# lzhLab/kmcEx

Hardware: AMD Instinct MI355X
Metric: k-mers/s encoded (insert) + k-mers/s queried, k=31 nh=7; % HBM-BW roofline (higher is better)
Workload: dtype u64; 1 GPU; synthetic 100000000 distinct canonical 31-mers per GPU, D1 counts, insert then query (110000000 queries: all inserted k-mers shuffled, half reverse-complemented, +10% absent); k=31, nh=7, nb=5, ci=1, cs=1023, kmers_per_gpu=100000000

## Files before the change

### kmcex_amd/csrc/kernels.hip

```cpp
#include "launchers.h"
#include <cstdlib>

__constant__ u32 c_seeds[128] = {
	46757, 46769, 46771, 46807, 46811, 46817, 46819, 46829, 46831, 46853, 46861, 46867, 46877, 46889, 46901, 46919,
	46933, 46957, 46993, 46997, 47017, 47041, 47051, 47057, 47059, 47087, 47093, 47111, 47119, 47123, 47129, 47137,
	47143, 47147, 47149, 47161, 47189, 47207, 47221, 47237, 47251, 47269, 47279, 47287, 47293, 47297, 47303, 47309,
	47317, 47339, 47351, 47353, 47363, 47381, 47387, 47389, 47407, 47417, 47419, 47431, 47441, 47459, 47491, 47497,
	47501, 47507, 47513, 47521, 47527, 47533, 47543, 47563, 47569, 47581, 47591, 47599, 47609, 47623, 47629, 47639,
	47653, 47657, 47659, 47681, 47699, 47701, 47711, 47713, 47717, 47737, 47741, 47743, 47777, 47779, 47791, 47797,
	47807, 47809, 47819, 47837, 47843, 47857, 47869, 47881, 47903, 47911, 47917, 47933, 47939, 47947, 47951, 47963,
	47969, 47977, 47981, 48017, 48023, 48029, 48049, 48073, 48079, 48091, 48109, 48119, 48121, 48131, 48157, 48163};

template <int W> __device__ __forceinline__ void load_kmer(const u64 *base, u64 i, u64 *v)
{
#pragma unroll
	for (int w = 0; w < W; w++) v[w] = base[i * W + w];
}
template <int W> __device__ __forceinline__ void store_kmer(u64 *base, u64 i, const u64 *v)
{
#pragma unroll
	for (int w = 0; w < W; w++) base[i * W + w] = v[w];
}

template <int W> __device__ __forceinline__ void bloom_insert_pm(const Premixed<W> &pm, const StrGeom g, u32 *bits, const ModU64 md, int nhash)
// ... 1700 lines not shown

template <int PW> __device__ __forceinline__ int decode_array(const ModelDev &md, const StrGeom gf, const Premixed<PW> &pf, int a)
{
	if (!md.km_mod.d) return -1;
	const cell_t *cells = md.cells[a];
	int v = 0;
	bool ok = true;
	for (int j = 0; j < md.nh && ok; j++) {
		u64 pos = mod_u64(murmur_seeded<PW>(pf, gf, c_seeds[(a * md.nh + j) & 127]), md.km_mod);
		const cell_t cell = cells[pos >> 4];
		u32 b = bit_in_cell(pos);
		ok = (cell >> (16 + b)) & 1u;
		v |= (int)((cell >> b) & 1u) << j;
	}
	return ok ? v : -1;
}

template <int PW> __device__ __forceinline__ int candidate_from_filters(const ModelDev &md, const StrGeom gf, const StrGeom gb, const Premixed<PW> &pf, const Premixed<PW> &pb)
{
	int occ = check_all_bf<PW>(md, gf, gb, pf, pb);
	if (occ != 0) return occ;
	if (bloom_check_pm<PW>(pb, gb, md.km_back, md.km_back_mod, md.nh - 2)) {
		int result = -1;
		for (int a = 0; a < md.nb; a++) {
			int d = decode_array<PW>(md, gf, pf, a);
			if (d >= 0) { result = d; if (d != 0) break; }
		}
		if (result > -1) return result;
	}
	return -2;
}

template <int PW, typename NEIGH>
__device__ __forceinline__ int occ_from_filters(const ModelDev &md, const StrGeom gf, const StrGeom gb, const Premixed<PW> &pf, const Premixed<PW> &pb, NEIGH neighbours)
{
	const bool in_back = bloom_check_pm<PW>(pb, gb, md.km_back, md.km_back_mod, md.nh - 2);
	const int occ = check_all_bf<PW>(md, gf, gb, pf, pb);
	if (!in_back) return occ;
	int nv = 0, first = 0;
	for (int a = 0; a < md.nb; a++) {
		int d = decode_array<PW>(md, gf, pf, a);
		if (d > 0) { if (nv == 0) first = d; nv++; }
	}
	int bin;
	if (nv == 0) bin = occ;
	else if (nv == 1) {
		bin = first;
		if (occ) {
			int cand[8];
			int nc = neighbours(cand), cnt = 0;
			for (int c = 0; c < 8; c++) cnt += (c < nc && cand[c] < md.ci + md.bf_num) ? 1 : 0;
			if (cnt >= nc / 2) bin = occ;
		}
	} else {
		int cand[8];
		int nc = neighbours(cand);
		if (nc <= 0) bin = 0;
		else {
			int min_dist = 2 << 20;
			bin = first;
			for (int a = 0; a < md.nb; a++) {
				int d = decode_array<PW>(md, gf, pf, a);
				if (d <= 0) continue;
				int cur = 2 << 20;
				for (int c = 0; c < 8; c++)
					if (c < nc) { int dd = d > cand[c] ? d - cand[c] : cand[c] - d; cur = dd < cur ? dd : cur; }
				if (min_dist > cur) { min_dist = cur; bin = d; }
			}
		}
	}
	return bin < (1 << md.nh) ? (int)md.mean_of_bin[bin] : 0;
}

template <int W> __device__ __forceinline__ int neighbour_candidate(const ModelDev &md, u64 *nv)
{
	min_kmer<W>(nv, md.k);
	int r = rest_check<W>(md, nv);
	if (r > 0) return (int)md.bin_of_occ[r];
	Aligned<W> al = left_align<W>(nv, md.k);
	Premixed<W> pf = premix_string<W>(al, md.gfull);
	Premixed<W> pb = premix_string<W>(drop_first_base<W>(al), md.gback);
	return candidate_from_filters<W>(md, md.gfull, md.gback, pf, pb);
}

template <int W> __device__ __forceinline__ int neighbour_bins(const ModelDev &md, const u64 *v, int *cand)
{
	int nc = 0;
	const int k = md.k;
	for (int x = 0; x < 8; x++) {
		u64 nv[W];
		if (x < 4) {
			if (W == 1) nv[0] = ((v[0] << 2) | (u64)x) & (k == 32 ? ~0ULL : ((1ULL << (2 * k)) - 1));
			else {
				nv[0] = ((v[0] << 2) | (v[W - 1] >> 62)) & (k == 64 ? ~0ULL : ((1ULL << (2 * k - 64)) - 1));
				nv[W - 1] = (v[W - 1] << 2) | (u64)x;
			}
		} else {
			u64 X = (u64)(x - 4);
			if (W == 1) nv[0] = (v[0] >> 2) | (X << (2 * (k - 1)));
			else {
				nv[W - 1] = (v[W - 1] >> 2) | (v[0] << 62);
				nv[0] = (v[0] >> 2) | (X << (2 * (k - 1) - 64));
			}
		}
		int c = neighbour_candidate<W>(md, nv);
		if (c != -2) cand[nc++] = c;
	}
	return nc;
}

template <int W, bool ACCT> __device__ __forceinline__ void query_packed_one(const ModelDev &md, u64 *v, u64 *acct, int *dst)
{
	if (md.k & 31) v[0] &= (1ULL << (2 * (md.k & 31))) - 1;
	min_kmer<W>(v, md.k);
	int occ = rest_check<W>(md, v);
	if (occ != 0) { *dst = occ; return; }
	Aligned<W> al = left_align<W>(v, md.k);
	Premixed<W> pf = premix_string<W>(al, md.gfull);
	Premixed<W> pb = premix_string<W>(drop_first_base<W>(al), md.gback);
	*dst = occ_from_filters<W>(md, md.gfull, md.gback, pf, pb, [&](int *cand) { if (ACCT) atomicAdd(acct, 1ULL); return neighbour_bins<W>(md, v, cand); });
}

template <int W, bool ACCT> __global__ __launch_bounds__(256) void k_query(ModelDev md, const u64 *kmers, u64 n, int *out, u64 *acct)
{
	const u64 q = (u64)blockIdx.x * 256 + threadIdx.x;
	if (q >= n) return;
	u64 v[W];
	load_kmer<W>(kmers, q, v);
	query_packed_one<W, ACCT>(md, v, acct, out + q);
}

struct AStr { u64 b[8]; };

__device__ __forceinline__ u32 code_of_byte(u32 c) { return c == 'C' ? 1u : (c == 'G' ? 2u : (c == 'T' ? 3u : 0u)); }

__device__ __forceinline__ void astr_codes(const AStr &s, int L, u64 &hi, u64 &lo)
{
	hi = lo = 0;
#pragma unroll
	for (int w = 0; w < 8; w++)
#pragma unroll
		for (int j = 0; j < 8; j++)
			if (8 * w + j < L) {
				const u32 c = code_of_byte((u32)(s.b[w] >> (8 * j)) & 0xFFu);
				hi = (hi << 2) | (lo >> 62);
				lo = (lo << 2) | c;
			}
}
__device__ __forceinline__ void astr_clip(AStr &s, int L)
{
#pragma unroll
	for (int w = 0; w < 8; w++) {
		const int keep = L - 8 * w;
// ... 669 lines not shown
		else hipLaunchKernelGGL((k_kmback_emit<2, 16, 2>), grid, blk, 0, st, md, bd, kmers, surv, i0, istride, pp, n_in_block, bs);
	}
}
void bs_apply(const BitScatter &bs, hipStream_t st)
{
	if (!bs.cap2) { hipLaunchKernelGGL(k_bs_apply, dim3(BS_BINS), dim3(1024), 0, st, bs); return; }
	const unsigned per_bin = (bs.cap + 256 * BS_SPLIT_K - 1) / (256 * BS_SPLIT_K);
	hipLaunchKernelGGL(k_bs_split, dim3(per_bin < 64 ? per_bin : 64, BS_BINS), dim3(256), 0, st, bs);
	hipLaunchKernelGGL(k_bs_apply2, dim3(1u << (bs.wshift - bs.tlog2), BS_BINS), dim3(1024), 0, st, bs);
}

void kmc_decode(const KmcDecode &d, int W_, u64 rec0, u64 n, u64 *kmers, u32 *counts, hipStream_t st)
{
	if (!n) return;
	DISPATCH_W(W_, hipLaunchKernelGGL(k_kmc_decode<W>, dim3((unsigned)((n + 255) / 256)), dim3(256), 0, st, d, rec0, n, kmers, counts));
}

void ring_import(const ModelDev &md, const BlockDev &bd, int pp, const RingLists &rl, u64 *stg_kmers, u32 *stg_counts, hipStream_t st)
{
	DISPATCH_W(words(md), hipLaunchKernelGGL(k_ring_import<W>, dim3(KMX_BUCKET / 256, md.nb), dim3(256), 0, st, bd, md.nb, pp, rl, stg_kmers, stg_counts));
}
void ring_export(const ModelDev &md, const BlockDev &bd, int pp, const RingLists &rl, u64 *feedback, hipStream_t st)
{
	DISPATCH_W(words(md), hipLaunchKernelGGL(k_ring_export<W>, dim3(KMX_BUCKET / 256, md.nb), dim3(256), 0, st, bd, pp, rl, feedback));
}
void or_words(u32 *dst, const u32 *src, u64 n, hipStream_t st)
{
	if (!n) return;
	u64 blocks = (n + 1023) / 1024;
	if (blocks > 65536) blocks = 65536;
	hipLaunchKernelGGL(k_or_words, dim3((unsigned)blocks), dim3(256), 0, st, dst, src, n);
}

void query(const ModelDev &md, const u64 *kmers, u64 n, int *out, hipStream_t st, KernelProf *prof, u64 *acct)
{
	if (!n) return;
	KPROF_BEGIN(prof, KC_QUERY, st);
	if (acct) DISPATCH_W(words(md), hipLaunchKernelGGL((k_query<W, true>), dim3((unsigned)((n + 255) / 256)), dim3(256), 0, st, md, kmers, n, out, acct));
	else DISPATCH_W(words(md), hipLaunchKernelGGL((k_query<W, false>), dim3((unsigned)((n + 255) / 256)), dim3(256), 0, st, md, kmers, n, out, (u64 *)nullptr));
	KPROF_END(prof, st);
}

void query_ascii(const ModelDev &md, int L, const unsigned char *strs, int stride, u64 n, int *out, hipStream_t st)
{
	if (!n) return;
	const StrGeom gf = make_geom(L), gb = make_geom(L >= 2 ? L - 2 : 0);
	DISPATCH_W(words(md), hipLaunchKernelGGL(k_query_ascii<W>, dim3((unsigned)((n + 255) / 256)), dim3(256), 0, st, md, gf, gb, L, strs, stride, n, out));
}

void query_seq(const ModelDev &md, const unsigned char *seq, u64 n_bases, const u64 *offs, u64 n_seqs, u64 p0, u64 n_win, int *out, u32 *dlist, u32 cap, u32 *dcnt, u32 *dcnt_next, hipStream_t st, KernelProf *prof)
{
	if (!n_win) return;
	KPROF_BEGIN(prof, KC_QUERY, st);
	const StrGeom gf = make_geom(md.k), gb = make_geom(md.k - 2);
	DISPATCH_W(words(md), hipLaunchKernelGGL(k_query_seq<W>, dim3((unsigned)((n_win + SEQ_BT - 1) / SEQ_BT)), dim3(SEQ_BT), 0, st, md, seq, n_bases, offs, n_seqs, p0, n_win, out, dlist, cap, dcnt));
	DISPATCH_W(words(md), hipLaunchKernelGGL(k_query_ascii_at<W>, dim3(SEQ_DIRTY_WGS), dim3(256), 0, st, md, gf, gb, seq, n_bases, p0, (const u32 *)dlist, cap, (const u32 *)dcnt, dcnt_next, out));
	KPROF_END(prof, st);
}

void seq_summary_init(SeqSummary *rec, u64 n_seqs, hipStream_t st, KernelProf *prof)
{
	if (!n_seqs) return;
	KPROF_BEGIN(prof, KC_QUERY, st);
	hipLaunchKernelGGL(k_seq_summary_init, dim3((unsigned)((n_seqs + 255) / 256)), dim3(256), 0, st, rec, n_seqs);
	KPROF_END(prof, st);
}
// ... 65 lines not shown
```

### kmcex_amd/csrc/kmx_api.hip

```cpp
#include "../../include/kmx.h"
#include "hip_owned.h"
#include "kmc_reader.h"
#include "launchers.h"
#include "reads_reader.h"
#include "strpack.h"

#include <algorithm>
#include <atomic>
#include <exception>
#include <new>
#include <cstdarg>
#include <cstdio>
#include <cstdlib>
#include <cstring>
#include <chrono>
#include <condition_variable>
#include <functional>
#include <memory>
#include <mutex>
#include <string>
#include <thread>
#include <type_traits>
#include <vector>
#include <dlfcn.h>
// ... 58 lines not shown
	for (int i = 0; i < e1 && i < mc; i++) bin_of_occ[i] = i;
	mean_of_bin.assign(e3, 0);
	for (int b = 0; b < e1; b++) mean_of_bin[b] = b;
	std::vector<char> seen(e3, 0);
	for (int i = e1; i < mc; i++) {
		u32 b = bin_of_occ[i];
		if (b < (u32)e3 && !seen[b]) { seen[b] = 1; if ((int)b >= e1) mean_of_bin[b] = mean_of_occ[i]; }
	}
	return 0;
}

static int kmx_occubin_impl(int cs, int nh, uint32_t *bin_of_occ, uint32_t *mean_of_bin)
{
	if (nh < 3 || nh > KMX_MAX_NH || cs < 1) return fail(KMX_E_ARG, "bad cs/nh");
	std::vector<u32> b, m;
	if (occubin_tables(cs, nh, b, m)) return fail(KMX_E_ARG, "cs=%d too small for nh=%d", cs, nh);
	memcpy(bin_of_occ, b.data(), b.size() * 4);
	memcpy(mean_of_bin, m.data(), m.size() * 4);
	return KMX_OK;
}

struct RestTable {
	int k = 0, pre_len = 0, map_size = 0, pre_buffer_size = 0, suff_group = 0;
	u64 suff_bin_size = 0, entries = 0;
	std::vector<int> hash2index, pre_buffer, count_bin;
	std::vector<unsigned char> suffix_bin;
	bool host_valid = false;
	DevBuf<int> d_h2i, d_pre, d_cnt;
	DevBuf<u64> d_suf;
	DevBuf<u64> d_sorted;
	int fbits = 0;
	DevBuf<u32> d_fine;
	DevBuf<u64> d_q;
	void reset_dev() { d_h2i.reset(); d_pre.reset(); d_cnt.reset(); d_suf.reset(); d_sorted.reset(); d_fine.reset(); d_q.reset(); }
};
static int rest_prefix_len(int k) { for (int i = 7; i >= 3; i--) if ((k - i) % 4 == 0) return i; return 3; }
static int check_model_k(int k)
{
	if (k < 4 || k > 64) return fail(KMX_E_ARG, "k=%d out of range [4,64]%s", k, k == 3 ? ": the reference's rest table is undefined at k = 3 (prefix of 7 bases, rest.hpp:78-83)" : "");
	return KMX_OK;
}

struct RestEnt { u64 w[2]; int c; };

enum { ST_EMPTY = 0, ST_BUILDING = 1, ST_READY = 2 };

struct kmx_model {
	int ci = 1, cs = 1023, nh = 7, nb = 5, k = 0, bf_num = 1, W = 1;
	int device = 0, state = ST_EMPTY;
	hipStream_t stream = nullptr;
	std::vector<u32> h_bin_of_occ, h_mean_of_bin;
	DevBuf<u32> d_bin_of_occ, d_mean_of_bin;
	u64 n_total = 0, n_km = 0, n_bf[3] = {0, 0, 0};
	u64 byte_bf[3] = {0, 0, 0}, byte_bf_back[3] = {0, 0, 0}, km_byte_size = 0, byte_km_back = 0, ncells = 0;
	DevBuf<u32> d_bloom;
	u64 bloom_words = 0, bf_woff[3] = {0, 0, 0}, bf_back_woff[3] = {0, 0, 0};
	u32 *d_bf[3] = {nullptr, nullptr, nullptr}, *d_bf_back[3] = {nullptr, nullptr, nullptr};
	DevBuf<u32> d_km_back;
	DevBuf<cell_t> d_cells[KMX_MAX_NB];
	RestTable rest;
	ModelDev md;
	DevBuf<u64> d_stg_kmers;
	DevBuf<u32> d_stg_counts;
	u64 stg_n = 0;
	BlockDev bd;
	DevBuf<unsigned char> d_block_scratch;
	int scratch_nb = 0, scratch_W = 0;
// ... 274 lines not shown
	m->n_km = m->n_total - nbf;
	m->km_byte_size = (m->n_km >> 4) * (u64)m->nh;
	m->byte_km_back = (m->n_km >> 4) * (u64)(m->nh - 2);
	m->ncells = (m->km_byte_size + 1) / 2;
}

static void fill_model_dev(kmx_model *m)
{
	ModelDev &md = m->md;
	memset(&md, 0, sizeof md);
	md.k = m->k; md.nh = m->nh; md.nb = m->nb; md.ci = m->ci; md.cs = m->cs; md.bf_num = m->bf_num;
	{
		const char *e = hook_env("KMX_NH_FIRST"), *e2 = hook_env("KMX_NH_SECOND");
		const int f = e ? atoi(e) : (2 * m->nh + 3) / 7, f2 = e2 ? atoi(e2) : (4 * m->nh + 3) / 7;
		md.nh_first = f < 1 ? 1 : (f > m->nh ? m->nh : f);
		md.nh_second = f2 < md.nh_first ? md.nh_first : (f2 > m->nh ? m->nh : f2);
	}
	md.gfull = make_geom(m->k);
	md.gback = make_geom(m->k - 2);
	for (int i = 0; i < 3; i++) {
		md.bf[i] = m->d_bf[i]; md.bf_mod[i] = make_mod(i < m->bf_num ? m->byte_bf[i] * 8 : 0);
		md.bf_back[i] = m->d_bf_back[i]; md.bf_back_mod[i] = make_mod(i < m->bf_num ? m->byte_bf_back[i] * 8 : 0);
	}
	md.km_back = m->d_km_back; md.km_back_mod = make_mod(m->byte_km_back * 8);
	md.kmb_direct = m->kmb_deferred ? 0 : 1;
	md.bloom_direct = m->blm_deferred ? 0 : 1;
	for (int i = 0; i < 3; i++) { md.bf_woff[i] = m->bf_woff[i]; md.bf_back_woff[i] = m->bf_back_woff[i]; }
	for (int a = 0; a < m->nb; a++) md.cells[a] = m->d_cells[a];
	md.km_mod = make_mod(m->km_byte_size * 8);
	md.bin_of_occ = m->d_bin_of_occ; md.mean_of_bin = m->d_mean_of_bin;
	md.rest_pre_len = m->rest.pre_len; md.rest_W = m->W; md.rest_entries = m->rest.entries;
	md.rest_h2i = m->rest.d_h2i; md.rest_pre = m->rest.d_pre; md.rest_suf = m->rest.d_suf; md.rest_cnt = m->rest.d_cnt;
	md.rest_fbits = m->rest.fbits; md.rest_fine = m->rest.d_fine; md.rest_q = m->rest.d_q;
}

static int alloc_arrays(kmx_model *m)
{
	m->rest.reset_dev();
	{
		u64 off = 0;
		for (int i = 0; i < 3; i++) {
			m->bf_woff[i] = off; off += i < m->bf_num ? (m->byte_bf[i] + 3) / 4 + 1 : 0;
			m->bf_back_woff[i] = off; off += i < m->bf_num ? (m->byte_bf_back[i] + 3) / 4 + 1 : 0;
		}
		m->bloom_words = off;
		TRY(ensure(m->d_bloom, off + 1, true, m->stream));
		for (int i = 0; i < 3; i++) {
			m->d_bf[i] = i < m->bf_num ? m->d_bloom + m->bf_woff[i] : nullptr;
			m->d_bf_back[i] = i < m->bf_num ? m->d_bloom + m->bf_back_woff[i] : nullptr;
		}
	}
	TRY(ensure(m->d_km_back, (m->byte_km_back + 3) / 4 + 1, true, m->stream));
	for (int a = 0; a < m->nb; a++) TRY(ensure(m->d_cells[a], m->ncells + 1, true, m->stream));
	return KMX_OK;
}

static const u32 kBsMaxTileShift = 3;
static u64 bs_cap_hook()
{
	static const u64 v = [] { const char *e = hook_env("KMX_BS_CAP"); const long long x = e ? atoll(e) : 0; return x > 0 ? (u64)std::min<long long>(x, 1 << 18) : 0ull; }();
	return v;
}
static u32 bs_tile_log2()
{
	const char *e = hook_env("KMX_BS_TILE_LOG2");
	const int x = e ? atoi(e) : 20;
	return (u32)std::min(std::max(x, 10), 20);
}
static int bs_geometry(kmx_model *m, BitScatter &bs, u64 nwords, u64 cap, bool *ok)
{
	*ok = false;
// ... 153 lines not shown
	for (int s2 = 0; s2 < KMX_NSLOW; s2++) bd.Urec[s2] = (u64 *)(base + o_U[s2]);
	bd.Un = (int *)(base + o_Un); bd.R = (u64 *)(base + o_R);
	bd.tile_cnt[0] = (int *)(base + o_tc0); bd.tile_cnt[1] = (int *)(base + o_tc1);
	bd.surv = (unsigned char *)(base + o_surv);
	m->d_surv[0] = bd.surv; m->d_surv[1] = (unsigned char *)(base + o_surv1);
	for (int q = 0; q < 2; q++) {
		bd.uw[q] = (u32 *)(base + o_uw[q]); bd.crec[q] = (u32 *)(base + o_crec[q]);
		bd.cl_tup[q] = (u64 *)(base + o_cl_tup[q]); bd.cl_cnt[q] = (int *)(base + o_cl_cnt[q]);
	}
	bd.cl_ovf = (int *)(base + o_cl_ovf);
	bd.stats = m->d_stats;
	TRY(dalloc(m->d_rest_n, 1, false, m->stream));
	TRY(dalloc(m->d_stale_kmers, (u64)nb * 2, false, m->stream));
	TRY(dalloc(m->d_stale_counts, (u64)nb, false, m->stream));
	TRY(dalloc(m->d_total, 4, true, m->stream));
	return KMX_OK;
}

static int kmx_begin_impl(kmx_model *m, int k, const uint64_t n_bf[3], uint64_t n_total)
{
	if (!m) return fail(KMX_E_ARG, "null model");
	TRY(check_model_k(k));
	HIPCHK(hipSetDevice(m->device));
	if (!m->cnt.building) free_count(m, true);
	u64 s = 0;
	for (int i = 0; i < m->bf_num; i++) s += n_bf[i];
	if (s > n_total) return fail(KMX_E_ARG, "n_bf exceeds n_total");
	m->k = k; m->W = (k + 31) / 32;
	m->n_total = n_total;
	for (int i = 0; i < 3; i++) m->n_bf[i] = i < m->bf_num ? n_bf[i] : 0;
	compute_sizes(m);
	if (m->d_block_scratch && (m->scratch_nb != m->nb || m->scratch_W != m->W)) free_build_state(m);
	TRY(alloc_arrays(m));
	m->rest = RestTable();
	TRY(setup_kmback_scatter(m));
	TRY(setup_bloom_scatter(m));
	bs_attach_level2(m);
	fill_model_dev(m);
	const int nb = m->nb;
	const u64 B = KMX_BUCKET, blk = (u64)nb * B;
	if (!m->d_block_scratch) {
		const int rc = alloc_build_state(m);
		if (rc) { m->d_block_scratch.reset(); return rc; }
	}
	m->stg_n = 0;
	for (int q = 0; q < 2; q++) HIPCHK(hipMemsetAsync(m->bd.cl_cnt[q], 0, (u64)nb * KMX_CL_MAXBINS * 4, m->stream));
	HIPCHK(hipMemsetAsync(m->bd.dfail, 0, blk, m->stream));
	HIPCHK(hipMemsetAsync(m->bd.cl_ovf, 0, (u64)nb * 4, m->stream));
	m->pp = 0; m->pending = false; m->pending_t = 0;
	m->defer = !m->dbg_no_defer && m->km_byte_size * 8 <= (1ULL << KMX_CL_MIX_BITS);
	const u64 want_rest = std::max<u64>(m->n_km / 8, 2 * blk) + blk;
	if (m->d_rest_counts.cap() < want_rest || !m->d_rest_kmers) {
		m->d_rest_kmers.reset(); m->d_rest_counts.reset();
		TRY(dalloc(m->d_rest_kmers, want_rest * m->W, false, m->stream));
		TRY(dalloc(m->d_rest_counts, want_rest, false, m->stream));
	}
	m->rest_upper = 0;
	HIPCHK(hipMemsetAsync(m->d_rest_n, 0, 8, m->stream));
	HIPCHK(hipMemsetAsync(m->d_stale_kmers, 0, (u64)nb * 16, m->stream));
	HIPCHK(hipMemsetAsync(m->d_stale_counts, 0, (u64)nb * 4, m->stream));
	HIPCHK(hipMemsetAsync(m->d_stats, 0, ST_N * 8, m->stream));
	m->blocks = 0; m->rounds = 0;
	m->h_feedback[0] = ~0ULL; m->h_feedback[1] = 0; m->h_feedback[2] = (u64)KMX_BUCKET * (u64)m->nh / KMX_CL_MAXBINS / 4;
	{
		const double L = (double)m->km_byte_size * 8.0;
		const double p = L > 0 ? std::min(1.0, (double)m->nh * m->nh * 131072.0 / L) : 1.0;
		const double u0 = 157000.0 * p;
// ... 227 lines not shown
	HIPCHK(F.ensure(F.HOST | F.DEV, B, 0, W, 0));
	auto drain = scope_exit([&] { hipStreamSynchronize(F.copy); hipStreamSynchronize(m->stream); });
	HIPCHK(hipEventRecord(F.ev_free[0], m->stream));
	HIPCHK(hipEventRecord(F.ev_free[1], m->stream));
	auto stage = [&](int s, uint64_t lo, uint64_t c) -> int {
		HIPCHK(hipEventSynchronize(F.ev_copied[s]));
		parallel_copy(F.km[s], kmers + lo * W, c * W * 8);
		parallel_copy(F.cnt[s], counts + lo, c * 4);
		HIPCHK(hipStreamWaitEvent(F.copy, F.ev_free[s], 0));
		HIPCHK(hipMemcpyAsync(F.dk[s], F.km[s], c * W * 8, hipMemcpyHostToDevice, F.copy));
		HIPCHK(hipMemcpyAsync(F.dc[s], F.cnt[s], c * 4, hipMemcpyHostToDevice, F.copy));
		HIPCHK(hipEventRecord(F.ev_copied[s], F.copy));
		return KMX_OK;
	};
	TRY(stage(0, 0, std::min<uint64_t>(B, n)));
	int s = 0;
	for (uint64_t done = 0; done < n; s ^= 1) {
		const uint64_t c = std::min<uint64_t>(B, n - done), next = done + c;
		if (next < n) TRY(stage(s ^ 1, next, std::min<uint64_t>(B, n - next)));
		HIPCHK(hipStreamWaitEvent(m->stream, F.ev_copied[s], 0));
		TRY(kmx_insert_batch_dev(m, (const uint64_t *)F.dk[s].get(), F.dc[s], c));
		HIPCHK(hipEventRecord(F.ev_free[s], m->stream));
		done = next;
	}
	return KMX_OK;
}

static int rest_to_device(kmx_model *m);
static int rest_build_accel(kmx_model *m);

static int build_rest(kmx_model *m, u64 n)
{
	RestTable &r = m->rest;
	r.reset_dev();
	const int W = m->W, k = m->k;
	r.k = k;
	r.pre_len = rest_prefix_len(k);
	r.map_size = 1 << (2 * r.pre_len);
	r.suff_group = (k - r.pre_len) / 4;
	r.entries = n;
	r.suff_bin_size = n * (u64)r.suff_group;
	r.host_valid = false;
	HIPCHK(r.d_sorted.alloc(n * W + 2));
	HIPCHK(r.d_cnt.alloc(n + 4));
	HIPCHK(r.d_suf.alloc(n * W + 2));
	HIPCHK(r.d_h2i.alloc((u64)r.map_size));
	HIPCHK(r.d_pre.alloc((u64)r.map_size + 2));
	HIPCHK(hipMemsetAsync(r.d_h2i, 0xFF, (u64)r.map_size * 4, m->stream));
	KPROF_BEGIN(&m->prof, KC_REST, m->stream);
	HIPCHK(kmxk::rest_sort(m->d_rest_kmers, m->d_rest_counts, n, W, k, r.d_sorted, r.d_cnt, m->stream));
	HIPCHK(kmxk::rest_index(r.d_sorted, n, W, k, r.pre_len, r.d_h2i, r.d_pre, r.d_suf, m->d_total, m->stream));
	KPROF_END(&m->prof, m->stream);
	HIPCHK(hipMemcpyAsync(m->h_total, m->d_total, 4, hipMemcpyDeviceToHost, m->stream));
	HIPCHK(hipStreamSynchronize(m->stream));
	r.pre_buffer_size = *m->h_total + 1;
	return rest_build_accel(m);
}

static int rest_build_accel(kmx_model *m)
{
	RestTable &r = m->rest;
	int F = 1;
	while ((1ULL << F) < r.entries * 2 && F < 26) F++;
	F = std::max(F, 2 * r.pre_len);
	F = std::min(F, 2 * r.k);
	r.fbits = F;
	HIPCHK(r.d_fine.alloc((1ULL << F) + 2));
	HIPCHK(r.d_q.alloc((u64)r.map_size * m->W));
	kmxk::rest_accel(r.d_sorted, r.entries, m->W, r.k, F, r.d_h2i, r.d_pre, r.d_suf, r.map_size, r.d_fine, r.d_q, m->stream);
	HIPCHK(hipGetLastError());
	return KMX_OK;
}

static int rest_materialize_host(kmx_model *m)
{
	RestTable &r = m->rest;
	if (r.host_valid) return KMX_OK;
	const u64 n = r.entries;
	r.hash2index.resize(r.map_size); r.pre_buffer.resize(r.pre_buffer_size); r.count_bin.resize(n);
	r.suffix_bin.assign(r.suff_bin_size, 0);
	HIPCHK(hipMemcpy(r.hash2index.data(), r.d_h2i, (u64)r.map_size * 4, hipMemcpyDeviceToHost));
	HIPCHK(hipMemcpy(r.pre_buffer.data(), r.d_pre, (u64)r.pre_buffer_size * 4, hipMemcpyDeviceToHost));
	if (n) {
		DevBuf<unsigned char> d_bytes;
		HIPCHK(d_bytes.alloc(r.suff_bin_size));
		kmxk::rest_suffix_bytes(r.d_sorted, n, m->W, r.suff_group, d_bytes, m->stream);
		hipError_t e = hipMemcpyAsync(r.suffix_bin.data(), d_bytes, r.suff_bin_size, hipMemcpyDeviceToHost, m->stream);
		if (e == hipSuccess) e = hipMemcpyAsync(r.count_bin.data(), r.d_cnt, n * 4, hipMemcpyDeviceToHost, m->stream);
		if (e == hipSuccess) e = hipStreamSynchronize(m->stream);
		if (e != hipSuccess) return fail(KMX_E_NODEVICE, "rest table download failed");
	}
	r.host_valid = true;
	return KMX_OK;
}

static int rest_to_device(kmx_model *m)
{
	RestTable &r = m->rest;
	const int W = m->W;
	const u64 n = r.entries;
	std::vector<u64> suf(n * W + 1, 0);
	for (u64 e = 0; e < n; e++) {
		unsigned __int128 val = 0;
// ... 1558 lines not shown
```

### kmcex_amd/csrc/kmx_types.h

```cpp
#pragma once
#include "device_common.h"

struct ModelDev {
	int k, nh, nb, ci, cs, bf_num;
	int nh_first, nh_second;
	StrGeom gfull, gback;
	u32 *bf[3];      ModU64 bf_mod[3];
	u32 *bf_back[3]; ModU64 bf_back_mod[3];
	u32 *km_back;    ModU64 km_back_mod;
	cell_t *cells[KMX_MAX_NB];
	ModU64 km_mod;
	int bloom_direct;
	u64 bf_woff[3], bf_back_woff[3];
	int kmb_direct;
	const u32 *bin_of_occ;
	const u32 *mean_of_bin;
	int rest_pre_len, rest_W;
	u64 rest_entries;
	const int *rest_h2i;
	const int *rest_pre;
	const u64 *rest_suf;
	const int *rest_cnt;
	int rest_fbits;
	const u32 *rest_fine;
	const u64 *rest_q;
};

#define BS_BINS 256
#define BS_TILE_WORDS (1u << 15)
struct BitScatter {
	u32 *words;
	u64 nwords;
	u32 wshift;
	u32 cap;
	u32 *tup;
	int *cnt;
	u32 tlog2;
	u32 cap2;
	u32 *tup2;
	int *cnt2;
};
struct KmbackJob {
	const u64 *kmers;
	const unsigned char *surv;
	int n_in_block;
	int i0, n_lists;
};
#define BS_MAX_TILES_LOG2 8

struct KmcDecode {
	const unsigned char *recs;
	const u64 *lut;
	u64 n_lut, prefix_mask;
	u32 rec_bytes, suf_bytes, cnt_bytes;
};

enum { ST_ATTEMPTS = 0, ST_SUCCESSES, ST_SLOW_SUCC, ST_CONTENDED, ST_FIN_ITERS, ST_BAD_COUNT, ST_MAX_U0, ST_MAX_UFIN,
       ST_PIPE_ATTEMPTS, ST_PIPE_SUCC,
// ... 149 lines not shown
```

### kmcex_amd/csrc/launchers.h

```cpp
#pragma once
#include "kmx_types.h"

template <typename T> struct DevBuf;

namespace kmxk {
void histogram(const u32 *, u64, int, int, int, u64 *, u64 *, hipStream_t);
int classify_tiles(u64 n);
void classify_count(const ModelDev &, const u64 *, const u32 *, u64, u64, int *, int *, int *, u64 *, const BitScatter &, int, hipStream_t, KernelProf *);
void classify_scatter(const ModelDev &, const u64 *, const u32 *, u64, const int *, u64 *, u32 *, u64, hipStream_t);
void block_init(const BlockDev &, int, int, int, hipStream_t);
void round(const ModelDev &, const BlockDev &, int, int, int, u64 *, int, hipStream_t, KernelProf *, const KmbackJob *, const BitScatter *, const RoundProbe *probe = nullptr);
void commit_flush(const ModelDev &, const BlockDev &, int, int, hipStream_t, KernelProf *);
void rest_append(const ModelDev &, const BlockDev &, int, int, int, u64 *, int *, unsigned long long *, u64 *, int *, u64 *, hipStream_t, int istride = 1);
void kmback_emit(const ModelDev &, const BlockDev &, const u64 *, const unsigned char *, int, int, int, int, int, const BitScatter &, hipStream_t, int istride = 1);
void bs_apply(const BitScatter &, hipStream_t);
void ring_import(const ModelDev &, const BlockDev &, int, const RingLists &, u64 *, u32 *, hipStream_t);
void ring_export(const ModelDev &, const BlockDev &, int, const RingLists &, u64 *, hipStream_t);
void or_words(u32 *, const u32 *, u64, hipStream_t);
void range_emit(const ModelDev &, const BlockDev &, const RangeDev &, const RangePlan &, int, int, bool, hipStream_t);
void range_seal(const RangeDev &, const RangePlan &, hipStream_t);
void range_verdict(const ModelDev &, const BlockDev &, int *, int, const RangeIn &, unsigned char *, int, bool, hipStream_t);
void range_apply(const ModelDev &, const BlockDev &, const RangeDev &, const RangePlan &, int, int, bool, hipStream_t);
void range_resolve(const ModelDev &, const BlockDev &, const RangeDev &, const RangePlan &, int, int, bool, hipStream_t);
void range_commit_apply(const ModelDev &, const RangeIn &, int, hipStream_t);
void query(const ModelDev &, const u64 *, u64, int *, hipStream_t, KernelProf *, u64 *acct = nullptr);
void query_ascii(const ModelDev &, int, const unsigned char *, int, u64, int *, hipStream_t);
void query_seq(const ModelDev &, const unsigned char *, u64, const u64 *, u64, u64, u64, int *, u32 *, u32, u32 *, u32 *, hipStream_t, KernelProf *);
void seq_summary_init(SeqSummary *, u64, hipStream_t, KernelProf *);
void seq_summary_finish(SeqSummary *, const u64 *, u64, u64, int, hipStream_t, KernelProf *);
void summarise_seq(const ModelDev &, const unsigned char *, u64, u64, const u64 *, u64, u64, u64, const SeqSumDev &, u32 *, u32, u32 *, u32 *, hipStream_t, KernelProf *);
void seq_correction_init(SeqCorrection *, const u64 *, u64, u64, int, hipStream_t, KernelProf *);
void correct_piece(const ModelDev &, const unsigned char *, u64, u64, u64, const u64 *, u64, u64, u64, u64, u64, u64 *, const CorrDev &, unsigned char *, u32 *, u32, u32 *, u32 *, hipStream_t, KernelProf *);
void cells_from_disk(const unsigned char *, const unsigned char *, u64, cell_t *, u64, hipStream_t);
void cells_to_disk(const cell_t *, u64, u64, int, unsigned char *, hipStream_t);
void debug_hash(int, const u64 *, u64, const u32 *, int, int, u64 *, hipStream_t);
void debug_min_kmer(int, const u64 *, u64, u64 *, hipStream_t);
void debug_mod(const u64 *, u64, u64, u64 *, hipStream_t);
void micro(int, u64 *, u64, u64, u64, u64 *, hipStream_t);
hipError_t rest_sort(const u64 *, const int *, u64, int, int, u64 *, int *, hipStream_t);
hipError_t rest_index(const u64 *, u64, int, int, int, int *, int *, u64 *, int *, hipStream_t);
void rest_expand(const int *, const int *, const u64 *, int, int, int, int, u64 *, hipStream_t);
void rest_accel(const u64 *, u64, int, int, int, const int *, const int *, const u64 *, int, u32 *, u64 *, hipStream_t);
void rest_suffix_bytes(const u64 *, u64, int, int, unsigned char *, hipStream_t);
void count_windows(int, const unsigned char *, u64, const u64 *, u64, u64, u64, u64 *, u64 *, u64, unsigned long long *, hipStream_t);
void kmc_decode(const KmcDecode &, int, u64, u64, u64 *, u32 *, hipStream_t);
hipError_t count_piece(int, int, u64 *, u64 *, u64, u64, u32 *, unsigned long long *, DevBuf<unsigned char> &tmp, hipStream_t);
hipError_t count_merge(int, const u64 *, const u32 *, u64, const u64 *, const u32 *, u64, u64 *, u32 *, DevBuf<unsigned char> &tmp, hipStream_t);
hipError_t count_reduce(int, const u64 *, const u32 *, u64, u64 *, u32 *, unsigned long long *, DevBuf<unsigned char> &tmp, hipStream_t);
hipError_t count_filter(int, const u64 *, const u32 *, u64, u32, u32, u32, u64 *, u32 *, unsigned char *, unsigned long long *, DevBuf<unsigned char> &tmp, hipStream_t);
}
```

### kmcex_amd/csrc/rest_device.hip

```cpp
#include "hip_owned.h"
#include "launchers.h"
#include <cstring>
#include <rocprim/rocprim.hpp>

namespace {

__global__ __launch_bounds__(256) void k_iota(u32 *idx, u64 n)
{
	u64 i = (u64)blockIdx.x * 256 + threadIdx.x;
	if (i < n) idx[i] = (u32)i;
}
__global__ __launch_bounds__(256) void k_split2(const u64 *km, u64 n, u64 *hi, u64 *lo)
{
	u64 i = (u64)blockIdx.x * 256 + threadIdx.x;
	if (i < n) { hi[i] = km[2 * i]; lo[i] = km[2 * i + 1]; }
}
__global__ __launch_bounds__(256) void k_gather_u64(const u64 *src, const u32 *idx, u64 n, u64 *dst)
{
	u64 i = (u64)blockIdx.x * 256 + threadIdx.x;
	if (i < n) dst[i] = src[idx[i]];
}
__global__ __launch_bounds__(256) void k_gather_final2(const u64 *km, const int *cnt, const u32 *idx, u64 n, u64 *okm, int *ocnt)
{
	u64 i = (u64)blockIdx.x * 256 + threadIdx.x;
// ... 62 lines not shown
		const u64 mid = (lo + hi) >> 1;
		const unsigned __int128 v = W == 1 ? (unsigned __int128)km[mid] : (((unsigned __int128)km[2 * mid] << 64) | km[2 * mid + 1]);
		if (v < thr) lo = mid + 1; else hi = mid;
	}
	fine[b] = (u32)lo;
}

__global__ __launch_bounds__(256) void k_next_first(const int *h2i, const int *pre, const u64 *suf, u64 n, int map_size, int W, u64 *q)
{
	int P = blockIdx.x * 256 + threadIdx.x;
	if (P >= map_size) return;
	const int g = h2i[P];
	u64 e = g >= 0 ? (u64)pre[g + 1] : n;
	for (int w = 0; w < W; w++) q[(u64)P * W + w] = e < n ? suf[e * W + w] : ~0ULL;
}

inline unsigned nblk(u64 n) { return (unsigned)((n + 255) / 256); }

}

__global__ __launch_bounds__(256) void k_rest_suffix_bytes(const u64 *km, u64 n, int W, int suff_group, unsigned char *out)
{
	const u64 e = (u64)blockIdx.x * 256 + threadIdx.x;
	if (e >= n) return;
	const u64 lo = km[e * W + (W - 1)], hi = W == 2 ? km[e * W] : 0;
	for (int g = 0; g < suff_group; g++) {
		const int sh = 8 * (suff_group - 1 - g);
		out[e * (u64)suff_group + g] = (unsigned char)(sh >= 64 ? hi >> (sh - 64) : lo >> sh);
	}
}

namespace kmxk {

hipError_t rest_sort(const u64 *km_in, const int *cnt_in, u64 n, int W, int k, u64 *km_out, int *cnt_out, hipStream_t st)
{
	if (!n) return hipSuccess;
	size_t tmp_bytes = 0;
	DevBuf<unsigned char> tmp;
	if (W == 1) {
		RCHK(rocprim::radix_sort_pairs(nullptr, tmp_bytes, km_in, km_out, cnt_in, cnt_out, n, 0, 2 * k, st));
		RCHK(tmp.alloc(tmp_bytes));
		hipError_t e = rocprim::radix_sort_pairs(tmp.get(), tmp_bytes, km_in, km_out, cnt_in, cnt_out, n, 0, 2 * k, st);
		hipStreamSynchronize(st);
		return e;
	}
	DevBuf<u64> hi, lo, key2, key3;
	DevBuf<u32> i0, i1;
	RCHK(hi.alloc(n)); RCHK(lo.alloc(n));
	RCHK(key2.alloc(n)); RCHK(key3.alloc(n));
	RCHK(i0.alloc(n)); RCHK(i1.alloc(n));
	hipLaunchKernelGGL(k_split2, dim3(nblk(n)), dim3(256), 0, st, km_in, n, hi.get(), lo.get());
	hipLaunchKernelGGL(k_iota, dim3(nblk(n)), dim3(256), 0, st, i0.get(), n);
	size_t t1 = 0, t2 = 0;
	RCHK(rocprim::radix_sort_pairs(nullptr, t1, lo.get(), key2.get(), i0.get(), i1.get(), n, 0, 64, st));
	RCHK(rocprim::radix_sort_pairs(nullptr, t2, key2.get(), key3.get(), i1.get(), i0.get(), n, 0, 2 * k - 64, st));
	tmp_bytes = t1 > t2 ? t1 : t2;
	RCHK(tmp.alloc(tmp_bytes));
	hipError_t e = rocprim::radix_sort_pairs(tmp.get(), tmp_bytes, lo.get(), key2.get(), i0.get(), i1.get(), n, 0, 64, st);
	if (e == hipSuccess) {
		hipLaunchKernelGGL(k_gather_u64, dim3(nblk(n)), dim3(256), 0, st, (const u64 *)hi.get(), (const u32 *)i1.get(), n, key2.get());
		e = rocprim::radix_sort_pairs(tmp.get(), tmp_bytes, key2.get(), key3.get(), i1.get(), i0.get(), n, 0, 2 * k - 64, st);
	}
	if (e == hipSuccess) hipLaunchKernelGGL(k_gather_final2, dim3(nblk(n)), dim3(256), 0, st, km_in, cnt_in, (const u32 *)i0.get(), n, km_out, cnt_out);
	hipStreamSynchronize(st);
	return e;
}

hipError_t rest_index(const u64 *km_sorted, u64 n, int W, int k, int pre_len, int *h2i, int *pre, u64 *suf, int *groups, hipStream_t st)
{
	const int sbits = 2 * (k - pre_len);
	RCHK(hipMemsetAsync(groups, 0, 4, st));
	RCHK(hipMemsetAsync(pre, 0, 4, st));
	if (!n) return hipSuccess;
	DevBuf<int> flag, scan;
	DevBuf<unsigned char> tmp;
	size_t tmp_bytes = 0;
	RCHK(flag.alloc(n));
	RCHK(scan.alloc(n));
	hipLaunchKernelGGL(k_rest_flags, dim3(nblk(n)), dim3(256), 0, st, km_sorted, n, W, sbits, flag.get(), suf);
	RCHK(rocprim::inclusive_scan(nullptr, tmp_bytes, flag.get(), scan.get(), n, rocprim::plus<int>(), st));
	RCHK(tmp.alloc(tmp_bytes));
	hipError_t e = rocprim::inclusive_scan(tmp.get(), tmp_bytes, flag.get(), scan.get(), n, rocprim::plus<int>(), st);
	if (e == hipSuccess) hipLaunchKernelGGL(k_rest_index, dim3(nblk(n)), dim3(256), 0, st, km_sorted, n, W, sbits, (const int *)flag.get(), (const int *)scan.get(), h2i, pre, groups);
	hipStreamSynchronize(st);
	return e;
}

void rest_expand(const int *h2i, const int *pre, const u64 *suf, int map_size, int W, int k, int pre_len, u64 *out, hipStream_t st)
{
	hipLaunchKernelGGL(k_rest_expand, dim3(nblk(map_size)), dim3(256), 0, st, h2i, pre, suf, map_size, W, 2 * (k - pre_len), out);
}

void rest_accel(const u64 *km_sorted, u64 n, int W, int k, int F, const int *h2i, const int *pre, const u64 *suf, int map_size, u32 *fine, u64 *q, hipStream_t st)
{
	const u64 nbuckets = 1ULL << F;
	hipLaunchKernelGGL(k_fine_index, dim3(nblk(nbuckets + 1)), dim3(256), 0, st, km_sorted, n, W, 2 * k - F, nbuckets, fine);
	hipLaunchKernelGGL(k_next_first, dim3(nblk(map_size)), dim3(256), 0, st, h2i, pre, suf, n, map_size, W, q);
}

void rest_suffix_bytes(const u64 *km_sorted, u64 n, int W, int suff_group, unsigned char *out, hipStream_t st)
{
	if (n) hipLaunchKernelGGL(k_rest_suffix_bytes, dim3(nblk(n)), dim3(256), 0, st, km_sorted, n, W, suff_group, out);
}

}
```

Measured before the change: 1.504 billion k-mers/s.

## Interleave rest-table hint bits with km_back filter to skip rest lookups

Builds a combined 64-bit-word array where the low half mirrors the km_back Bloom filter and the high half holds a Bloom-style hint of the k-mers stored in the rest table (rows and phantom prefixes). At query time a single pass over those words answers both the km_back membership test and whether the rest table could contain the k-mer, so the rest_check lookup is skipped for most queries. The rest build also reuses persistent scratch buffers instead of allocating per call and drops intermediate stream syncs. The cost is extra memory for the interleaved array, extra build kernels, and a slightly more complex query path.

```diff
diff --git a/kmcex_amd/csrc/kernels.hip b/kmcex_amd/csrc/kernels.hip
--- a/kmcex_amd/csrc/kernels.hip
+++ b/kmcex_amd/csrc/kernels.hip
@@ -1756,9 +1756,8 @@
 }
 
 template <int PW, typename NEIGH>
-__device__ __forceinline__ int occ_from_filters(const ModelDev &md, const StrGeom gf, const StrGeom gb, const Premixed<PW> &pf, const Premixed<PW> &pb, NEIGH neighbours)
-{
-	const bool in_back = bloom_check_pm<PW>(pb, gb, md.km_back, md.km_back_mod, md.nh - 2);
+__device__ __forceinline__ int occ_from_filters_ib(const ModelDev &md, const StrGeom gf, const StrGeom gb, const Premixed<PW> &pf, const Premixed<PW> &pb, const bool in_back, NEIGH neighbours)
+{
 	const int occ = check_all_bf<PW>(md, gf, gb, pf, pb);
 	if (!in_back) return occ;
 	int nv = 0, first = 0;
@@ -1794,6 +1793,12 @@
 		}
 	}
 	return bin < (1 << md.nh) ? (int)md.mean_of_bin[bin] : 0;
+}
+template <int PW, typename NEIGH>
+__device__ __forceinline__ int occ_from_filters(const ModelDev &md, const StrGeom gf, const StrGeom gb, const Premixed<PW> &pf, const Premixed<PW> &pb, NEIGH neighbours)
+{
+	const bool in_back = bloom_check_pm<PW>(pb, gb, md.km_back, md.km_back_mod, md.nh - 2);
+	return occ_from_filters_ib<PW>(md, gf, gb, pf, pb, in_back, neighbours);
 }
 
 template <int W> __device__ __forceinline__ int neighbour_candidate(const ModelDev &md, u64 *nv)
@@ -1837,12 +1842,66 @@
 {
 	if (md.k & 31) v[0] &= (1ULL << (2 * (md.k & 31))) - 1;
 	min_kmer<W>(v, md.k);
+	auto neighbours = [&](int *cand) { if (ACCT) atomicAdd(acct, 1ULL); return neighbour_bins<W>(md, v, cand); };
+	if (md.kmq) {
+		Aligned<W> al = left_align<W>(v, md.k);
+		Premixed<W> pb = premix_string<W>(drop_first_base<W>(al), md.gback);
+		bool kb_ok = true, hint_ok = true;
+		for (int j = 0; j < md.nh - 2 && (kb_ok || hint_ok); j++) {
+			const u64 pos = mod_u64(murmur_seeded<W>(pb, md.gback, c_seeds[j]), md.km_back_mod);
+			const u64 x = md.kmq[pos >> 5];
+			const u32 b = bit_in_word32(pos);
+			kb_ok = kb_ok && (((u32)x >> b) & 1u);
+			hint_ok = hint_ok && (((u32)(x >> 32) >> b) & 1u);
+		}
+		const int occ = hint_ok ? rest_check<W>(md, v) : 0;
+		if (occ != 0) { *dst = occ; return; }
+		Premixed<W> pf = premix_string<W>(al, md.gfull);
+		*dst = occ_from_filters_ib<W>(md, md.gfull, md.gback, pf, pb, kb_ok, neighbours);
+		return;
+	}
 	int occ = rest_check<W>(md, v);
 	if (occ != 0) { *dst = occ; return; }
 	Aligned<W> al = left_align<W>(v, md.k);
 	Premixed<W> pf = premix_string<W>(al, md.gfull);
 	Premixed<W> pb = premix_string<W>(drop_first_base<W>(al), md.gback);
-	*dst = occ_from_filters<W>(md, md.gfull, md.gback, pf, pb, [&](int *cand) { if (ACCT) atomicAdd(acct, 1ULL); return neighbour_bins<W>(md, v, cand); });
+	*dst = occ_from_filters<W>(md, md.gfull, md.gback, pf, pb, neighbours);
+}
+
+__global__ __launch_bounds__(256) void k_kmq_fill(const u32 *km_back, u64 nwords, u64 *kmq)
+{
+	const u64 w = (u64)blockIdx.x * 256 + threadIdx.x;
+	if (w < nwords) kmq[w] = km_back[w];
+}
+template <int W> __device__ __forceinline__ void rest_hint_set(const ModelDev &md, u64 *kmq, const u64 *v)
+{
+	Premixed<W> pb = premix_string<W>(drop_first_base<W>(left_align<W>(v, md.k)), md.gback);
+	for (int j = 0; j < md.nh - 2; j++) {
+		const u64 pos = mod_u64(murmur_seeded<W>(pb, md.gback, c_seeds[j]), md.km_back_mod);
+		u32 *w = (u32 *)(kmq + (pos >> 5)) + 1;
+		atomicOr(w, 1u << bit_in_word32(pos));
+	}
+}
+template <int W> __global__ __launch_bounds__(256) void k_rest_hint_rows(ModelDev md, const u64 *sorted, u64 n, u64 *kmq)
+{
+	const u64 e = (u64)blockIdx.x * 256 + threadIdx.x;
+	if (e >= n) return;
+	u64 v[W];
+	load_kmer<W>(sorted, e, v);
+	rest_hint_set<W>(md, kmq, v);
+}
+template <int W> __global__ __launch_bounds__(256) void k_rest_hint_phantoms(ModelDev md, const int *h2i, const u64 *q, int map_size, u64 *kmq)
+{
+	const int P = blockIdx.x * 256 + threadIdx.x;
+	if (P >= map_size || h2i[P] < 0) return;
+	u64 v[W];
+	load_kmer<W>(q, (u64)P, v);
+	if (v[0] == ~0ULL) return;
+	const int sbits = 2 * (md.k - md.rest_pre_len);
+	if (W == 1) v[0] |= (u64)P << sbits;
+	else if (sbits >= 64) v[0] |= (u64)P << (sbits - 64);
+	else { v[0] |= (u64)P >> (64 - sbits); v[W - 1] |= (u64)P << sbits; }
+	rest_hint_set<W>(md, kmq, v);
 }
 
 template <int W, bool ACCT> __global__ __launch_bounds__(256) void k_query(ModelDev md, const u64 *kmers, u64 n, int *out, u64 *acct)
@@ -2578,6 +2637,14 @@
 	hipLaunchKernelGGL(k_or_words, dim3((unsigned)blocks), dim3(256), 0, st, dst, src, n);
 }
 
+void rest_hint(const ModelDev &md, u64 km_words, const u64 *sorted, u64 n, const int *h2i, const u64 *q, int map_size, u64 *kmq, hipStream_t st)
+{
+	hipLaunchKernelGGL(k_kmq_fill, dim3((unsigned)((km_words + 255) / 256)), dim3(256), 0, st, (const u32 *)md.km_back, km_words, kmq);
+	if (!n) return;
+	DISPATCH_W(words(md), hipLaunchKernelGGL(k_rest_hint_rows<W>, dim3((unsigned)((n + 255) / 256)), dim3(256), 0, st, md, sorted, n, kmq));
+	DISPATCH_W(words(md), hipLaunchKernelGGL(k_rest_hint_phantoms<W>, dim3((unsigned)((map_size + 255) / 256)), dim3(256), 0, st, md, h2i, q, map_size, kmq));
+}
+
 void query(const ModelDev &md, const u64 *kmers, u64 n, int *out, hipStream_t st, KernelProf *prof, u64 *acct)
 {
 	if (!n) return;
diff --git a/kmcex_amd/csrc/kmx_api.hip b/kmcex_amd/csrc/kmx_api.hip
--- a/kmcex_amd/csrc/kmx_api.hip
+++ b/kmcex_amd/csrc/kmx_api.hip
@@ -114,7 +114,16 @@
 	int fbits = 0;
 	DevBuf<u32> d_fine;
 	DevBuf<u64> d_q;
-	void reset_dev() { d_h2i.reset(); d_pre.reset(); d_cnt.reset(); d_suf.reset(); d_sorted.reset(); d_fine.reset(); d_q.reset(); }
+	DevBuf<u64> d_kmq;
+	bool kmq_valid = false;
+	DevBuf<unsigned char> d_tmp;
+	void clear()
+	{
+		k = pre_len = map_size = pre_buffer_size = suff_group = fbits = 0;
+		suff_bin_size = entries = 0;
+		hash2index.clear(); pre_buffer.clear(); count_bin.clear(); suffix_bin.clear();
+		host_valid = kmq_valid = false;
+	}
 };
 static int rest_prefix_len(int k) { for (int i = 7; i >= 3; i--) if ((k - i) % 4 == 0) return i; return 3; }
 static int check_model_k(int k)
@@ -455,11 +464,12 @@
 	md.rest_pre_len = m->rest.pre_len; md.rest_W = m->W; md.rest_entries = m->rest.entries;
 	md.rest_h2i = m->rest.d_h2i; md.rest_pre = m->rest.d_pre; md.rest_suf = m->rest.d_suf; md.rest_cnt = m->rest.d_cnt;
 	md.rest_fbits = m->rest.fbits; md.rest_fine = m->rest.d_fine; md.rest_q = m->rest.d_q;
+	md.kmq = m->rest.kmq_valid ? m->rest.d_kmq.get() : nullptr;
 }
 
 static int alloc_arrays(kmx_model *m)
 {
-	m->rest.reset_dev();
+	m->rest.kmq_valid = false;
 	{
 		u64 off = 0;
 		for (int i = 0; i < 3; i++) {
@@ -679,7 +689,7 @@
 	compute_sizes(m);
 	if (m->d_block_scratch && (m->scratch_nb != m->nb || m->scratch_W != m->W)) free_build_state(m);
 	TRY(alloc_arrays(m));
-	m->rest = RestTable();
+	m->rest.clear();
 	TRY(setup_kmback_scatter(m));
 	TRY(setup_bloom_scatter(m));
 	bs_attach_level2(m);
@@ -973,7 +983,6 @@
 static int build_rest(kmx_model *m, u64 n)
 {
 	RestTable &r = m->rest;
-	r.reset_dev();
 	const int W = m->W, k = m->k;
 	r.k = k;
 	r.pre_len = rest_prefix_len(k);
@@ -982,20 +991,22 @@
 	r.entries = n;
 	r.suff_bin_size = n * (u64)r.suff_group;
 	r.host_valid = false;
-	HIPCHK(r.d_sorted.alloc(n * W + 2));
-	HIPCHK(r.d_cnt.alloc(n + 4));
-	HIPCHK(r.d_suf.alloc(n * W + 2));
-	HIPCHK(r.d_h2i.alloc((u64)r.map_size));
-	HIPCHK(r.d_pre.alloc((u64)r.map_size + 2));
+	r.kmq_valid = false;
+	HIPCHK(r.d_sorted.ensure(n * W + 2, m->stream));
+	HIPCHK(r.d_cnt.ensure(n + 4, m->stream));
+	HIPCHK(r.d_suf.ensure(n * W + 2, m->stream));
+	HIPCHK(r.d_h2i.ensure((u64)r.map_size, m->stream));
+	HIPCHK(r.d_pre.ensure((u64)r.map_size + 2, m->stream));
 	HIPCHK(hipMemsetAsync(r.d_h2i, 0xFF, (u64)r.map_size * 4, m->stream));
 	KPROF_BEGIN(&m->prof, KC_REST, m->stream);
-	HIPCHK(kmxk::rest_sort(m->d_rest_kmers, m->d_rest_counts, n, W, k, r.d_sorted, r.d_cnt, m->stream));
-	HIPCHK(kmxk::rest_index(r.d_sorted, n, W, k, r.pre_len, r.d_h2i, r.d_pre, r.d_suf, m->d_total, m->stream));
+	HIPCHK(kmxk::rest_sort(m->d_rest_kmers, m->d_rest_counts, n, W, k, r.d_sorted, r.d_cnt, r.d_tmp, m->stream));
+	HIPCHK(kmxk::rest_index(r.d_sorted, n, W, k, r.pre_len, r.d_h2i, r.d_pre, r.d_suf, m->d_total, r.d_tmp, m->stream));
 	KPROF_END(&m->prof, m->stream);
 	HIPCHK(hipMemcpyAsync(m->h_total, m->d_total, 4, hipMemcpyDeviceToHost, m->stream));
+	TRY(rest_build_accel(m));
 	HIPCHK(hipStreamSynchronize(m->stream));
 	r.pre_buffer_size = *m->h_total + 1;
-	return rest_build_accel(m);
+	return KMX_OK;
 }
 
 static int rest_build_accel(kmx_model *m)
@@ -1006,10 +1017,20 @@
 	F = std::max(F, 2 * r.pre_len);
 	F = std::min(F, 2 * r.k);
 	r.fbits = F;
-	HIPCHK(r.d_fine.alloc((1ULL << F) + 2));
-	HIPCHK(r.d_q.alloc((u64)r.map_size * m->W));
+	HIPCHK(r.d_fine.ensure((1ULL << F) + 2, m->stream));
+	HIPCHK(r.d_q.ensure((u64)r.map_size * m->W, m->stream));
 	kmxk::rest_accel(r.d_sorted, r.entries, m->W, r.k, F, r.d_h2i, r.d_pre, r.d_suf, r.map_size, r.d_fine, r.d_q, m->stream);
 	HIPCHK(hipGetLastError());
+	r.kmq_valid = false;
+	const char *hint = hook_env("KMX_REST_HINT");
+	if (m->byte_km_back && !(hint && hint[0] == '0')) {
+		const u64 km_words = (m->byte_km_back + 3) / 4 + 1;
+		HIPCHK(r.d_kmq.ensure(km_words, m->stream));
+		fill_model_dev(m);
+		kmxk::rest_hint(m->md, km_words, r.d_sorted, r.entries, r.d_h2i, r.d_q, r.map_size, r.d_kmq, m->stream);
+		HIPCHK(hipGetLastError());
+		r.kmq_valid = true;
+	}
 	return KMX_OK;
 }
 
diff --git a/kmcex_amd/csrc/kmx_types.h b/kmcex_amd/csrc/kmx_types.h
--- a/kmcex_amd/csrc/kmx_types.h
+++ b/kmcex_amd/csrc/kmx_types.h
@@ -24,6 +24,7 @@
 	int rest_fbits;
 	const u32 *rest_fine;
 	const u64 *rest_q;
+	const u64 *kmq;
 };
 
 #define BS_BINS 256
diff --git a/kmcex_amd/csrc/launchers.h b/kmcex_amd/csrc/launchers.h
--- a/kmcex_amd/csrc/launchers.h
+++ b/kmcex_amd/csrc/launchers.h
@@ -37,8 +37,9 @@
 void debug_min_kmer(int, const u64 *, u64, u64 *, hipStream_t);
 void debug_mod(const u64 *, u64, u64, u64 *, hipStream_t);
 void micro(int, u64 *, u64, u64, u64, u64 *, hipStream_t);
-hipError_t rest_sort(const u64 *, const int *, u64, int, int, u64 *, int *, hipStream_t);
-hipError_t rest_index(const u64 *, u64, int, int, int, int *, int *, u64 *, int *, hipStream_t);
+hipError_t rest_sort(const u64 *, const int *, u64, int, int, u64 *, int *, DevBuf<unsigned char> &tmp, hipStream_t);
+hipError_t rest_index(const u64 *, u64, int, int, int, int *, int *, u64 *, int *, DevBuf<unsigned char> &tmp, hipStream_t);
+void rest_hint(const ModelDev &, u64, const u64 *, u64, const int *, const u64 *, int, u64 *, hipStream_t);
 void rest_expand(const int *, const int *, const u64 *, int, int, int, int, u64 *, hipStream_t);
 void rest_accel(const u64 *, u64, int, int, int, const int *, const int *, const u64 *, int, u32 *, u64 *, hipStream_t);
 void rest_suffix_bytes(const u64 *, u64, int, int, unsigned char *, hipStream_t);
diff --git a/kmcex_amd/csrc/rest_device.hip b/kmcex_amd/csrc/rest_device.hip
--- a/kmcex_amd/csrc/rest_device.hip
+++ b/kmcex_amd/csrc/rest_device.hip
@@ -118,58 +118,55 @@
 
 namespace kmxk {
 
-hipError_t rest_sort(const u64 *km_in, const int *cnt_in, u64 n, int W, int k, u64 *km_out, int *cnt_out, hipStream_t st)
+struct Carve {
+	size_t total = 0;
+	size_t take(size_t bytes) { const size_t o = total; total += (bytes + 255) & ~(size_t)255; return o; }
+};
+
+hipError_t rest_sort(const u64 *km_in, const int *cnt_in, u64 n, int W, int k, u64 *km_out, int *cnt_out, DevBuf<unsigned char> &tmp, hipStream_t st)
 {
 	if (!n) return hipSuccess;
 	size_t tmp_bytes = 0;
-	DevBuf<unsigned char> tmp;
 	if (W == 1) {
 		RCHK(rocprim::radix_sort_pairs(nullptr, tmp_bytes, km_in, km_out, cnt_in, cnt_out, n, 0, 2 * k, st));
-		RCHK(tmp.alloc(tmp_bytes));
-		hipError_t e = rocprim::radix_sort_pairs(tmp.get(), tmp_bytes, km_in, km_out, cnt_in, cnt_out, n, 0, 2 * k, st);
-		hipStreamSynchronize(st);
-		return e;
+		RCHK(tmp.ensure(tmp_bytes, st));
+		return rocprim::radix_sort_pairs(tmp.get(), tmp_bytes, km_in, km_out, cnt_in, cnt_out, n, 0, 2 * k, st);
 	}
-	DevBuf<u64> hi, lo, key2, key3;
-	DevBuf<u32> i0, i1;
-	RCHK(hi.alloc(n)); RCHK(lo.alloc(n));
-	RCHK(key2.alloc(n)); RCHK(key3.alloc(n));
-	RCHK(i0.alloc(n)); RCHK(i1.alloc(n));
-	hipLaunchKernelGGL(k_split2, dim3(nblk(n)), dim3(256), 0, st, km_in, n, hi.get(), lo.get());
-	hipLaunchKernelGGL(k_iota, dim3(nblk(n)), dim3(256), 0, st, i0.get(), n);
 	size_t t1 = 0, t2 = 0;
-	RCHK(rocprim::radix_sort_pairs(nullptr, t1, lo.get(), key2.get(), i0.get(), i1.get(), n, 0, 64, st));
-	RCHK(rocprim::radix_sort_pairs(nullptr, t2, key2.get(), key3.get(), i1.get(), i0.get(), n, 0, 2 * k - 64, st));
+	RCHK(rocprim::radix_sort_pairs(nullptr, t1, km_in, km_out, (const u32 *)cnt_in, (u32 *)cnt_out, n, 0, 64, st));
+	RCHK(rocprim::radix_sort_pairs(nullptr, t2, km_in, km_out, (const u32 *)cnt_in, (u32 *)cnt_out, n, 0, 2 * k - 64, st));
 	tmp_bytes = t1 > t2 ? t1 : t2;
-	RCHK(tmp.alloc(tmp_bytes));
-	hipError_t e = rocprim::radix_sort_pairs(tmp.get(), tmp_bytes, lo.get(), key2.get(), i0.get(), i1.get(), n, 0, 64, st);
-	if (e == hipSuccess) {
-		hipLaunchKernelGGL(k_gather_u64, dim3(nblk(n)), dim3(256), 0, st, (const u64 *)hi.get(), (const u32 *)i1.get(), n, key2.get());
-		e = rocprim::radix_sort_pairs(tmp.get(), tmp_bytes, key2.get(), key3.get(), i1.get(), i0.get(), n, 0, 2 * k - 64, st);
-	}
-	if (e == hipSuccess) hipLaunchKernelGGL(k_gather_final2, dim3(nblk(n)), dim3(256), 0, st, km_in, cnt_in, (const u32 *)i0.get(), n, km_out, cnt_out);
-	hipStreamSynchronize(st);
-	return e;
+	Carve c;
+	const size_t o_hi = c.take(n * 8), o_lo = c.take(n * 8), o_key2 = c.take(n * 8), o_key3 = c.take(n * 8), o_i0 = c.take(n * 4), o_i1 = c.take(n * 4), o_tmp = c.take(tmp_bytes);
+	RCHK(tmp.ensure(c.total, st));
+	unsigned char *base = tmp.get();
+	u64 *hi = (u64 *)(base + o_hi), *lo = (u64 *)(base + o_lo), *key2 = (u64 *)(base + o_key2), *key3 = (u64 *)(base + o_key3);
+	u32 *i0 = (u32 *)(base + o_i0), *i1 = (u32 *)(base + o_i1);
+	hipLaunchKernelGGL(k_split2, dim3(nblk(n)), dim3(256), 0, st, km_in, n, hi, lo);
+	hipLaunchKernelGGL(k_iota, dim3(nblk(n)), dim3(256), 0, st, i0, n);
+	RCHK(rocprim::radix_sort_pairs(base + o_tmp, tmp_bytes, lo, key2, i0, i1, n, 0, 64, st));
+	hipLaunchKernelGGL(k_gather_u64, dim3(nblk(n)), dim3(256), 0, st, (const u64 *)hi, (const u32 *)i1, n, key2);
+	RCHK(rocprim::radix_sort_pairs(base + o_tmp, tmp_bytes, key2, key3, i1, i0, n, 0, 2 * k - 64, st));
+	hipLaunchKernelGGL(k_gather_final2, dim3(nblk(n)), dim3(256), 0, st, km_in, cnt_in, (const u32 *)i0, n, km_out, cnt_out);
+	return hipGetLastError();
 }
 
-hipError_t rest_index(const u64 *km_sorted, u64 n, int W, int k, int pre_len, int *h2i, int *pre, u64 *suf, int *groups, hipStream_t st)
+hipError_t rest_index(const u64 *km_sorted, u64 n, int W, int k, int pre_len, int *h2i, int *pre, u64 *suf, int *groups, DevBuf<unsigned char> &tmp, hipStream_t st)
 {
 	const int sbits = 2 * (k - pre_len);
 	RCHK(hipMemsetAsync(groups, 0, 4, st));
 	RCHK(hipMemsetAsync(pre, 0, 4, st));
 	if (!n) return hipSuccess;
-	DevBuf<int> flag, scan;
-	DevBuf<unsigned char> tmp;
 	size_t tmp_bytes = 0;
-	RCHK(flag.alloc(n));
-	RCHK(scan.alloc(n));
-	hipLaunchKernelGGL(k_rest_flags, dim3(nblk(n)), dim3(256), 0, st, km_sorted, n, W, sbits, flag.get(), suf);
-	RCHK(rocprim::inclusive_scan(nullptr, tmp_bytes, flag.get(), scan.get(), n, rocprim::plus<int>(), st));
-	RCHK(tmp.alloc(tmp_bytes));
-	hipError_t e = rocprim::inclusive_scan(tmp.get(), tmp_bytes, flag.get(), scan.get(), n, rocprim::plus<int>(), st);
-	if (e == hipSuccess) hipLaunchKernelGGL(k_rest_index, dim3(nblk(n)), dim3(256), 0, st, km_sorted, n, W, sbits, (const int *)flag.get(), (const int *)scan.get(), h2i, pre, groups);
-	hipStreamSynchronize(st);
-	return e;
+	RCHK(rocprim::inclusive_scan(nullptr, tmp_bytes, (const int *)h2i, pre, n, rocprim::plus<int>(), st));
+	Carve c;
+	const size_t o_flag = c.take(n * 4), o_scan = c.take(n * 4), o_tmp = c.take(tmp_bytes);
+	RCHK(tmp.ensure(c.total, st));
+	int *flag = (int *)(tmp.get() + o_flag), *scan = (int *)(tmp.get() + o_scan);
+	hipLaunchKernelGGL(k_rest_flags, dim3(nblk(n)), dim3(256), 0, st, km_sorted, n, W, sbits, flag, suf);
+	RCHK(rocprim::inclusive_scan(tmp.get() + o_tmp, tmp_bytes, flag, scan, n, rocprim::plus<int>(), st));
+	hipLaunchKernelGGL(k_rest_index, dim3(nblk(n)), dim3(256), 0, st, km_sorted, n, W, sbits, (const int *)flag, (const int *)scan, h2i, pre, groups);
+	return hipGetLastError();
 }
 
 void rest_expand(const int *h2i, const int *pre, const u64 *suf, int map_size, int W, int k, int pre_len, u64 *out, hipStream_t st)
```

Result: no change. 1.496 billion k-mers/s (-0.5%).
